# jacobwilliams/splpak

Measured on AMD Instinct MI355X. Metric: fitted points/sec (splcw) + evals/sec (splfe), 3-D 1e7 pts 64^3 nodes, higher is better.
Workload: dtype f64; 1 GPU; C3: 3-D splcw least-squares spline fit, 10000000 weighted scattered points (Park-Miller stream, seed 42), 64x64x64 nodes, xtrap=1, real64; ncol=262144, points_per_gpu=10000000, points_total=10000000, parallelism=single GPU, rccl_ranks=0, refine_steps=2

## Files before the change

### splpak_amd/csrc/ndchol.hip

```cpp
#include "ndstate.hpp"
#include <cstdlib>

namespace splpak {
namespace nd {

hipError_t nd_prefit(splpak_plan *p, hipStream_t st, void *user)
{
    NdState *s = static_cast<NdState *>(user);
    s->tail_pending = false;
    if (s->sch.staged_init && !s->dist) return hipSuccess;
    if (!s->str.sU || !s->ev.evPre || splpak::opt_get("SPLPAK_ND_NO_EARLY_CLEAR")) return hipSuccess;
    long long head = 0;
    if (p->gscratch == s->factor) head = p->gscratch_doubles < s->factor_doubles ? p->gscratch_doubles : s->factor_doubles;
    else if (p->gscratch >= s->factor && p->gscratch < s->factor + s->factor_doubles) return hipSuccess;
    if (head >= s->factor_doubles) return hipSuccess;
    hipError_t e = hipEventRecord(s->ev.evPre, st);
    if (e == hipSuccess) e = hipStreamWaitEvent(s->str.sU, s->ev.evPre, 0);
    const int clear_wgs = splpak::opt_get("SPLPAK_ND_CLEAR_WGS") ? atoi(splpak::opt_get("SPLPAK_ND_CLEAR_WGS")) : 128;
    if (e == hipSuccess) {
        if (clear_wgs > 0) {
            launch_clear(clear_wgs, s->factor + head, s->factor_doubles - head, s->str.sU);
            e = hipGetLastError();
        } else
            e = hipMemsetAsync(s->factor + head, 0, sizeof(double) * (size_t)(s->factor_doubles - head), s->str.sU);
// ... 8 lines not shown
hipError_t nd_assemble(splpak_plan *p, hipStream_t st, void *user)
{
    NdState *s = static_cast<NdState *>(user);
    hipError_t e = hipSuccess;
    if (s->sch.staged_init && !s->dist) {
        if (!s->sch.istarts.empty())
            for (int x : s->sch.istarts[0]) launch_init(s, p->g, p->nst, s->fac.init.l[(size_t)x][0], st);
        return hipGetLastError();
    }
    if (s->tail_pending) {
        if (s->head_doubles > 0) e = hipMemsetAsync(s->factor, 0, sizeof(double) * (size_t)s->head_doubles, st);
        if (e == hipSuccess) e = hipStreamWaitEvent(st, s->ev.evTail, 0);
        s->tail_pending = false;
    } else
        e = hipMemsetAsync(s->factor, 0, sizeof(double) * (size_t)s->factor_doubles, st);
    if (e != hipSuccess) return e;
    launch_assemble(s, p->g, p->nst, st);
    return hipGetLastError();
}

namespace {

struct FactorRun {
    splpak_plan *p;
    NdState *s;
    hipStream_t st, sP, sU, sR;
    int *info_dev;
    double *minpiv_dev;
    CholStats *stats;
    bool timing;
    int pin_rounds;
    int qnext = 0;
    int la_evt = -1;
    bool joined = false, comm_failed = false;
    void syrk(const JobTable<SyrkJob> &tab, const Launch &l, hipStream_t q, bool schur, bool pinned) { launch_syrk(s, tab, l, q, stats, timing, schur, pinned, qnext); }
    void begin();
    void dist_join();
    void potrf_step(const Launch &lp, int k, hipStream_t sC, bool reserved, hipEvent_t after);
    void stage_prep(int i);
    void chain_step(int stg, int k, bool pinned, bool pin_potrf, int prep);
    void root_stage(int stg);
    void run_stage(int i);
    hipError_t end();
};

void hop(hipEvent_t e, hipStream_t from, hipStream_t to) { (void)hipEventRecord(e, from); (void)hipStreamWaitEvent(to, e, 0); }

void zero_block(NdState *s, int x, hipStream_t q) { launch_zero(s->fac.zero, s->fac.zero.l[(size_t)x][0], q); }

void ensure_events(NdState *s, int steps)
{
    for (auto *v : {&s->ev.evT, &s->ev.evI, &s->ev.evW})
        while ((int)v->size() < steps) v->push_back(nd_event(s));
}

void FactorRun::begin()
{
    NdTree &t = s->t;
    if (timing) {
        if (!s->ev.f0) { s->ev.f0 = nd_event(s, true); s->ev.f1 = nd_event(s, true); }
        (void)hipEventRecord(s->ev.f0, st);
    }
    if (s->used && s->ev.evDone) (void)hipStreamWaitEvent(st, s->ev.evDone, 0);
    if (s->zlast_valid) (void)hipStreamWaitEvent(st, s->ev.evZlast, 0);
    if (!s->s_clean && !s->sch.sc.st.empty())
        for (int x : s->sch.starts[0]) zero_block(s, x, st);
    s->s_clean = false;
    if (s->queues) (void)hipMemsetAsync(s->queues, 0, sizeof(int) * ND_QSTRIDE * (size_t)s->nqueues, st);
// ... 46 lines not shown
void FactorRun::potrf_step(const Launch &lp, int k, hipStream_t sC, bool reserved, hipEvent_t after)
{
    if (!reserved) { launch_potrf(s, s->fac.potrf, lp, sC, info_dev, minpiv_dev); return; }
    if (after) (void)hipStreamWaitEvent(sR, after, 0);
    else hop(s->ev.evR0, sC, sR);
    launch_potrf(s, s->fac.potrf, lp, sR, info_dev, minpiv_dev);
    hop(s->ev.evI[(size_t)k], sR, sC);
}

void FactorRun::stage_prep(int i)
{
    for (int x : s->sch.starts[(size_t)i]) zero_block(s, x, sU);
    if (s->sch.staged_init && !s->dist)
        for (int x : s->sch.istarts[(size_t)i]) {
            launch_init(s, p->g, p->nst, s->fac.init.l[(size_t)x][0], sU);
            if (s->sch.sc.st[(size_t)x].dep < 0 && sU != sP) (void)hipEventRecord(s->ev.evP[(size_t)x], sU);
        }
}

void FactorRun::chain_step(int stg, int k, bool pinned, bool pin_potrf, int prep)
{
    FactorTables &F = s->fac;
    const size_t S = (size_t)stg, K = (size_t)k;
    hipStream_t sC = sP;
    const Launch &ls = F.schur.l[S][K], &lf0 = F.fin[0].l[S][K], &lf1 = F.fin[1].l[S][K];
    const bool ahead = pinned && k > 0 && la_evt == k - 1;
    potrf_step(F.potrf.l[S][K], k, sC, pinned && (pin_potrf || ahead), ahead ? s->ev.evW[(size_t)(k - 1)] : nullptr);
    launch_trsm(F.trsm, F.trsm.l[S][K], sC);
    if (prep >= 0) {
        hop(s->ev.evU, sC, sU);
        stage_prep(prep);
    }
    if ((ls.count || lf0.count || lf1.count) && sU != sC) hop(s->ev.evT[K], sC, sU);
    syrk(F.upd, F.upd.l[S][K], sC, false, pinned);
    if (s->sch.chain_la[S] && F.updr.l[S][K].count) {
        if (pinned) {
            (void)hipEventRecord(s->ev.evW[K], sC);
            la_evt = k;
        }
        syrk(F.updr, F.updr.l[S][K], sC, false, pinned);
    }
    syrk(F.updo, F.updo.l[S][K], sC, false, pinned);
    syrk(F.schur, ls, sU, true, pinned);
    syrk(F.fin[0], lf0, sU, true, pinned);
    syrk(F.fin[1], lf1, sU, true, pinned);
}

void FactorRun::root_stage(int stg)
{
    FactorTables &F = s->fac;
    const size_t S = (size_t)stg;
    const int steps = (int)F.potrf.l[S].size();
    ensure_events(s, steps);
    const bool pinned = sR != nullptr && s->nres > 0 && steps > 0 && (int)F.potrf.l[S][0].grid <= pin_rounds * s->nres;
    const bool la = s->sch.lookahead[S] != 0, la2 = s->sch.lookahead[S] == 2;
    for (int k = 0; k < steps; ++k) {
        if (!la) { chain_step(stg, k, pinned, true, -1); continue; }
        const size_t K = (size_t)k;
        const Launch &ltb = F.trsmb.l[S][K], &lur = F.updr.l[S][K];
        potrf_step(F.potrf.l[S][K], k, sP, pinned, nullptr);
        if (ltb.count) {
            if (sU != sP) {
                if (!pinned) (void)hipEventRecord(s->ev.evI[K], sP);
                (void)hipStreamWaitEvent(sU, s->ev.evI[K], 0);
            }
            launch_trsm(F.trsmb, ltb, sU);
        }
        if (!la2 && k > 0 && sU != sP) (void)hipStreamWaitEvent(sP, s->ev.evW[K - 1], 0);
        launch_trsm(F.trsm, F.trsm.l[S][K], sP);
        if (lur.count && sU != sP) hop(s->ev.evT[K], sP, sU);
        if (la2 && k > 0 && sU != sP) (void)hipStreamWaitEvent(sP, s->ev.evW[K - 1], 0);
        syrk(F.upd, F.upd.l[S][K], sP, false, pinned);
        syrk(F.updr, lur, sU, false, pinned);
        if (sU != sP) (void)hipEventRecord(s->ev.evW[K], sU);
    }
    if (sU != sP) hop(s->ev.evU, sU, sP);
}

void FactorRun::run_stage(int i)
{
    FactorTables &F = s->fac;
    const NdStage &S = s->sch.sc.st[(size_t)i];
    if (s->dist && !joined && S.depth <= s->sh.dcut - 1) dist_join();
    auto passes = [&](int k) { return F.schur.l[(size_t)i][(size_t)k].count || F.fin[0].l[(size_t)i][(size_t)k].count || F.fin[1].l[(size_t)i][(size_t)k].count; };
    const int steps = (int)F.potrf.l[(size_t)i].size();
    const bool prep_late = splpak::opt_get("SPLPAK_ND_PREP_EARLY") == nullptr;
    const bool defer = prep_late && i > 0 && i != s->sch.root_stage && sU != sP && steps >= 2 && !passes(0);
    if (i > 0) {
        if (!defer) stage_prep(i);
        if (s->sch.staged_init && !s->dist && S.dep < 0 && sU != sP) (void)hipStreamWaitEvent(sP, s->ev.evP[(size_t)i], 0);
    }
    if (s->sch.fused && S.dep >= 0 && sU != sP) (void)hipStreamWaitEvent(sP, s->ev.evF[(size_t)S.dep], 0);
    la_evt = -1;
    if (i == s->sch.root_stage) { root_stage(i); return; }
    ensure_events(s, steps);
    const bool pinned = sR != nullptr && s->nres > 0 && steps > 0 && ((int)F.potrf.l[(size_t)i][0].grid <= pin_rounds * s->nres || s->sch.chain_la[(size_t)i]);
    const bool unpin_first = splpak::opt_get("SPLPAK_ND_PIN_FIRST") == nullptr;
    bool pass_running = !unpin_first;
    for (int k = 0; k < steps; ++k) {
        chain_step(i, k, pinned, pass_running, k == 0 && defer ? i : -1);
        if (passes(k)) pass_running = true;
    }
    if (s->sch.fused) (void)hipEventRecord(s->ev.evF[(size_t)i], sU);
    else {
        if (sU != sP) hop(s->ev.evU, sU, sP);
// ... 29 lines not shown
    s->s_clean = true;
    (void)hipEventRecord(s->ev.evDone, st);
    s->used = true;
    hipError_t err = hipGetLastError();
    if (timing) {
        (void)hipEventRecord(s->ev.f1, st);
        (void)hipEventSynchronize(s->ev.f1);
        float ms = 0;
        (void)hipEventElapsedTime(&ms, s->ev.f0, s->ev.f1);
        stats->factor_ms = ms;
        for (size_t i = 0; i < (size_t)stats->syrk_launches; ++i) {
            if (hipEventElapsedTime(&ms, s->ev.evA[i], s->ev.evB[i]) == hipSuccess) stats->syrk_ms += ms;
            else (void)hipGetLastError();
        }
    }
    if (err != hipSuccess || top_err != hipSuccess) s->s_clean = false;
    if (comm_failed) return hipErrorUnknown;
    return top_err != hipSuccess ? top_err : err;
}

}

hipError_t nd_factor(splpak_plan *p, int *info_dev, double *minpiv_dev, hipStream_t st, void *user)
{
    NdState *s = static_cast<NdState *>(user);
    const bool timing = p->stats.enabled;
    p->stats = CholStats{};
    p->stats.enabled = timing;
    const bool serial = splpak::opt_get("SPLPAK_NO_LOOKAHEAD") != nullptr;
    FactorRun r{p, s, st, s->str.sP, s->str.sU, s->str.sR, info_dev, minpiv_dev, &p->stats, timing};
    if (serial) r.sP = r.sU = st;
    if (serial || splpak::opt_get("SPLPAK_NO_PANEL_CU")) r.sR = nullptr;
    r.pin_rounds = splpak::opt_get("SPLPAK_ND_PIN_ROUNDS") ? atoi(splpak::opt_get("SPLPAK_ND_PIN_ROUNDS")) : 1;
    r.begin();
    for (int i = 0; i < (int)s->sch.sc.st.size(); ++i) r.run_stage(i);
    return r.end();
}

hipError_t nd_solve(splpak_plan *p, double *x, double *tmp, hipStream_t st, void *user)
{
    (void)tmp;
    NdState *s = static_cast<NdState *>(user);
    NdTree &t = s->t;
    SolveTables &T = s->sol;
    const long long n = t.vec_doubles;
    launch_gather(n, s->rowsrc, x, s->V, st);
    bool comm_failed = false;
    if (s->dist && s->sh.rank != 0)
        for (int id : t.by_depth[(size_t)(s->sh.dcut - 1)]) {
            const NdFront &f = t.fr[(size_t)id];
            (void)hipMemsetAsync(s->V + f.vofs, 0, sizeof(double) * (size_t)f.fp, st);
        }
    const int dlow = s->mdist ? s->top.pt.dcut : 0;
    if (s->mdist) ++s->top.sgen;
    for (int d = t.maxdepth; d >= dlow; --d) {
        if (d < t.maxdepth)
            for (int sl = 0; sl < 2; ++sl) launch_map(T.map, T.map.l[(size_t)(d + 1)][(size_t)sl], false, st);
        if (s->dist && d == s->sh.dcut - 1)
            for (int id : t.by_depth[(size_t)d]) {
                const NdFront &f = t.fr[(size_t)id];
                if (plan_allreduce(p, s->V + f.vofs, f.fp, st) != 0) comm_failed = true;
            }
        const int steps = (int)T.mv.l[(size_t)d].size();
        for (int k = 0; k < steps; ++k) {
            launch_mv(T.mv, T.mv.l[(size_t)d][(size_t)k], st);
            launch_fwd(T.fwd, T.fwd.l[(size_t)d][(size_t)k], st);
// ... 78 lines not shown
```

### splpak_amd/csrc/ndjobs.hip

```cpp
#include "ndstate.hpp"
#include <algorithm>

namespace splpak {
namespace nd {

namespace {

void front_step_jobs(NdState *s, int stg, int id, int k, bool two_level)
{
    NdTree &t = s->t;
    FactorTables &F = s->fac;
    const NdFront &f = t.fr[(size_t)id];
    const bool la = s->sch.lookahead[(size_t)stg] != 0, la2 = s->sch.lookahead[(size_t)stg] == 2, cla = s->sch.chain_la[(size_t)stg] != 0;
    const int schur_kb = s->sch.schur_kb;
    const int g0 = (k / schur_kb) * schur_kb, gend = std::min(g0 + schur_kb, f.nsteps) - 1;
    double *panel = s->factor + s->poff[(size_t)id];
    double *diag = panel + (long long)k * 256 + (long long)k * 256 * f.ld;
    double *below = diag + 256;
    const int nrows = f.fp - (k + 1) * 256;
    double *i16 = s->inv16 + (long long)(s->lblk[(size_t)id] + k) * 4096;
    const int ncols = std::max(1, std::min(256, f.w - k * 256));
    F.potrf.push(PotrfJob{diag, i16, f.ld, f.own0 + k * 256, ncols});
    const int nc = (f.wp - (k + 1) * 256) / 64, nr = nrows / 64;
    if (nrows > 0) {
// ... 9 lines not shown
            tab.push(a, trapezoid_items(c, r));
        };
        auto split = [&](JobTable<SyrkJob> &rect_tab, int nin) {
            const int n4 = std::min(nin, 4);
            trapezoid(F.upd, n4, std::min(nr, 4));
            if (nr > 4) {
                SyrkJob r = proto;
                r.nc = n4; r.nr = nr; r.zinit = -4;
                rect_tab.push(r, (long long)n4 * (nr - 4));
            }
            if (nin > 4) {
                SyrkJob t2 = proto;
                t2.P = below + 256;
                t2.C = below + (long long)256 * f.ld + 256 + (long long)256 * f.ld;
                t2.nc = nin - 4; t2.nr = nr - 4;
                F.updr.push(t2, trapezoid_items(nin - 4, nr - 4));
            }
        };
        if (!la && two_level) {
            const int nc_in = std::min(nc, (gend - k) * 4);
            if (nc_in > 0 && cla) split(F.updr, nc_in);
            else if (nc_in > 0) trapezoid(F.upd, nc_in, nr);
            if (k == gend) {
                SyrkJob o = proto;
                o.P = panel + (long long)(k + 1) * 256 + (long long)g0 * 256 * f.ld;
                o.kb = k - g0 + 1;
                o.nc = nc; o.nr = nr;
                F.updo.push(o, trapezoid_items(nc, nr));
                F.updo.cur.flop += 2.0 * 64 * 64 * 256.0 * o.kb * (double)trapezoid_items(nc, nr);
            }
        } else if (!la)
            trapezoid(F.upd, nc, nr);
        else
            split(la2 ? F.upd : F.updr, nc);
    }
    const int ns = f.hp / 64;
    if (ns > 0 && k == gend) {
        const int kb = k - g0 + 1;
        const int ksl = (k == f.nsteps - 1) ? 4 * ((ncols + 15) / 16) : 64;
        const double jitems = (double)trapezoid_items(ns, ns) - (s->full_diag ? 0.0 : 0.375 * ns);
        const double jflop = 2.0 * 64 * 64 * (256.0 * (kb - 1) + 4.0 * ksl) * jitems;
        const bool boundary = s->mdist && f.depth == s->top.pt.dcut;
        if (s->sch.fused && k == f.nsteps - 1 && f.parent >= 0 && !boundary) {
            const NdFront &pf = t.fr[(size_t)f.parent];
            const int leaf = s->sch.needs[(size_t)id] ? 0 : 1;
            F.fin[f.slot].push(SyrkJob{panel + f.wp + (long long)g0 * 256 * f.ld, s_ptr(s, id), f.ld, s_ld(s, id), ns, ns, 0, kb, ksl, leaf, s->pmap + f.bofs,
                                       s->factor + s->poff[(size_t)f.parent], s_ptr(s, f.parent), pf.ld, s_ld(s, f.parent), pf.wp, f.h},
                               trapezoid_items(ns, ns));
            F.fin[f.slot].cur.flop += jflop;
        } else {
            F.schur.push(SyrkJob{panel + f.wp + (long long)g0 * 256 * f.ld, s_ptr(s, id), f.ld, s_ld(s, id), ns, ns, 0, kb, ksl, 0, nullptr, nullptr, nullptr, 0, 0, 0, 0},
                         trapezoid_items(ns, ns));
            F.schur.cur.flop += jflop;
        }
    }
}

bool stage_jobs(NdState *s, int stg)
{
    NdTree &t = s->t;
    FactorTables &F = s->fac;
    const std::vector<int> &ids = s->sch.sc.st[(size_t)stg].ids;
    F.zero.open();
    for (int id : ids) {
        const NdFront &f = t.fr[(size_t)id];
        if (f.hp == 0 || !s->sch.needs[(size_t)id]) continue;
        const int nt = f.hp / 64;
        F.zero.push(ZeroJob{s_ptr(s, id), s_ld(s, id), nt, 0}, trapezoid_items(nt, nt));
    }
    if (!F.zero.close((size_t)stg, 0)) return false;
    F.init.open();
    for (int id : ids)
        if (s->poff[(size_t)id] >= 0) F.init.push(InitJob{id, 0}, t.fr[(size_t)id].wp);
    if (!F.init.close((size_t)stg, 0)) return false;
    if (s->sch.sc.st[(size_t)stg].depth >= 1 && !s->sch.fused)
        for (int sl = 0; sl < 2; ++sl) {
            F.add.open();
            for (int id : ids) {
                const NdFront &f = t.fr[(size_t)id];
                if (f.slot != sl || f.h == 0) continue;
                const NdFront &p = t.fr[(size_t)f.parent];
                const int nt = f.hp / 64;
                F.add.push(AddJob{s_ptr(s, id), s->pmap + f.bofs, s->factor + s->poff[(size_t)f.parent], s_ptr(s, f.parent), s_ld(s, id), p.ld,
                                  s_ld(s, f.parent), f.h, nt, p.wp, 0},
                           trapezoid_items(nt, nt));
            }
            if (!F.add.close((size_t)stg, (size_t)sl)) return false;
        }
    return true;
}

bool nd_build_factor_jobs(NdState *s)
{
    NdTree &t = s->t;
    FactorTables &F = s->fac;
    const int nstage = (int)s->sch.sc.st.size();
    JobTable<SyrkJob> *const syrk[] = {&F.upd, &F.updr, &F.updo, &F.schur, &F.fin[0], &F.fin[1]};
    s->sch.lookahead.assign((size_t)nstage, 0);
    s->sch.chain_la.assign((size_t)nstage, 0);
    for_each_table(F, [&](auto &tab) { tab.l.assign((size_t)nstage, {}); });
    const bool two_level = splpak::opt_get("SPLPAK_ND_NO_OUTER") == nullptr;
    for (int stg = 0; stg < nstage; ++stg) {
        const std::vector<int> &ids = s->sch.sc.st[(size_t)stg].ids;
        int steps = 0;
        for (int id : ids) steps = std::max(steps, t.fr[(size_t)id].nsteps);
        bool any_schur = false;
        for (int id : ids) any_schur = any_schur || t.fr[(size_t)id].hp > 0;
        const bool la = !any_schur && steps >= 4 && !splpak::opt_get("SPLPAK_ND_NO_ROOT_LOOKAHEAD");
        const bool la2 = la && !(splpak::opt_get("SPLPAK_ND_ROOT_LA") && atoi(splpak::opt_get("SPLPAK_ND_ROOT_LA")) == 1);
        const int cla_blocks = splpak::opt_get("SPLPAK_ND_CHAIN_LA") ? atoi(splpak::opt_get("SPLPAK_ND_CHAIN_LA")) : 8;
        const bool cla = !la && two_level && steps >= 2 && (int)ids.size() <= cla_blocks && !s->mdist;
        s->sch.chain_la[(size_t)stg] = cla ? 1 : 0;
        s->sch.lookahead[(size_t)stg] = la ? (la2 ? 2 : 1) : 0;
        for (int k = 0; k < steps; ++k) {
            F.potrf.open(); F.trsm.open(); F.trsmb.open();
            for (auto *tab : syrk) tab->open();
            for (int id : ids)
                if (k < t.fr[(size_t)id].nsteps) front_step_jobs(s, stg, id, k, two_level);
            const size_t S = (size_t)stg, K = (size_t)k;
            if (!F.potrf.close(S, K) || !F.trsm.close(S, K) || !F.trsmb.close(S, K)) return false;
            for (auto *tab : syrk)
                if (!tab->close(S, K)) return false;
            F.upd.l[S][K].flop = 2.0 * 64 * 64 * 256 * (double)F.upd.l[S][K].grid;
            F.updr.l[S][K].flop = 2.0 * 64 * 64 * 256 * (double)F.updr.l[S][K].grid;
        }
        if (!stage_jobs(s, stg)) return false;
    }
    for (size_t id = 0; id < t.fr.size(); ++id) {
        const NdFront &f = t.fr[id];
        if (!s->mine.empty() && !s->mine[id]) continue;
        for (int k = 0; k < f.nsteps; ++k) {
            const double *diag = s->factor + s->poff[id] + (long long)k * 256 + (long long)k * 256 * f.ld;
            const long long lb = s->lblk[id] + k;
            F.trinv.host.push_back(TrinvJob{diag, s->inv16 + lb * 4096, s->dinv + lb * 65536, s->dinvt + lb * 65536, f.ld});
        }
    }
    F.ntrinv = (int)F.trinv.host.size();
    return true;
}

bool nd_build_solve_jobs(NdState *s)
{
    NdTree &t = s->t;
    SolveTables &T = s->sol;
    const int nd = t.maxdepth + 1;
    for_each_table(T, [&](auto &tab) { tab.l.assign((size_t)nd, {}); });
    long long part_max = 0;
    for (int d = 0; d < nd; ++d) {
        std::vector<int> ids;
        for (int id : t.by_depth[(size_t)d])
            if (s->mine.empty() || s->mine[(size_t)id]) ids.push_back(id);
        int steps = 0;
        for (int id : ids) steps = std::max(steps, t.fr[(size_t)id].nsteps);
        for (int k = 0; k < steps; ++k) {
            T.mv.open(); T.fwd.open(); T.dot.open(); T.bwd.open();
            long long partofs = 0;
// ... 187 lines not shown
```

### splpak_amd/csrc/ndkernels.hip

```cpp
#include "ndstate.hpp"
#include "chol_device.hpp"
#include <hip/hip_ext.h>
#include <cmath>
#include <type_traits>

namespace splpak {
namespace nd {

template <typename J, typename F>
__device__ __forceinline__ int find_job(const J *__restrict__ jobs, int njobs, int b, F &&first)
{
    int lo = 0, hi = njobs - 1;
    while (lo < hi) {
        const int mid = (lo + hi + 1) >> 1;
        if (first(jobs[mid]) <= b) lo = mid;
        else hi = mid - 1;
    }
    return lo;
}

__device__ __forceinline__ double *schur_tile(double *S, long long lds, int ti, int tj, long long &ld)
{
    if (lds >= 0) {
        ld = lds;
// ... 144 lines not shown
                const unsigned ci = nd_cu_index();
                if (resmap[ci >> 5] & (1u << (ci & 31))) skip = atomicAdd(&queue[1], 1) < margin ? 1 : 0;
                s_b[1] = skip;
                s_b[0] = skip ? 0 : atomicAdd(&queue[0], 1);
            }
            __syncthreads();
            if (s_b[1]) {
                __builtin_amdgcn_s_sleep(127);
                __builtin_amdgcn_s_sleep(127);
                return;
            }
            b = s_b[0];
        }
    }
    if constexpr (WGW > 1) b = b * WGW + (int)(threadIdx.x >> 6);
    if (b >= nitems) return;
    const int sub = SPLIT == 1 ? 0 : b % SPLIT;
    if (SPLIT > 1) b /= SPLIT;
    const int m0 = SPLIT == 1 ? 0 : (SPLIT == 4 ? sub : sub >> 2), n0 = SPLIT == 16 ? (sub & 3) : 0;
    const int ji = find_job(jobs, njobs, b, [](const SyrkJob &t) { return t.item0; });
    const SyrkJob j = jobs[ji];
    int tj, ti;
    if (!SCHUR && j.zinit < 0) {
        const int rb = -j.zinit, per = j.nr - rb, it = b - j.item0;
        tj = it / per;
        ti = rb + it - tj * per;
    } else if (xm && j.nc == j.nr)
        panel_decode(b - j.item0, j.nr, tj, ti);
    else
        trapezoid_decode(b - j.item0, j.nr, tj, ti);
    if (tj >= j.nc || ti >= j.nr) return;
    const bool diag = ti == tj;
    if (SPLIT == 16 && diag && n0 < m0) return;
    const int lane = threadIdx.x & 63, l15 = lane & 15, q = lane >> 4;
    constexpr bool COUNTED = !(SCHUR && SPLIT == 4);
    typedef __attribute__((address_space(1))) double gdouble;
    typedef __attribute__((address_space(1))) const int gint;
    typedef typename std::conditional<COUNTED, __attribute__((address_space(1))) const double, const double>::type opnd_t;
    typedef typename std::conditional<COUNTED, gdouble, double>::type ctile_t;
    opnd_t *__restrict__ pJ = (opnd_t *)(j.P + (long long)(tj * 64 + 16 * m0 + l15) + (long long)q * j.ldp);
    opnd_t *__restrict__ pI = (opnd_t *)(j.P + (long long)(ti * 64 + 16 * n0 + l15) + (long long)q * j.ldp);
    long long ldc;
    ctile_t *__restrict__ C = (ctile_t *)schur_tile(j.C, j.ldc, ti, tj, ldc);
    const long long ldp = j.ldp;
    constexpr bool SBASE = COUNTED && SPLIT == 4;
    typedef __attribute__((address_space(1))) const char gcchar;
    auto uniform = [](const double *p) {
        const unsigned long long a = (unsigned long long)p;
        const unsigned lo = __builtin_amdgcn_readfirstlane((unsigned)a), hi = __builtin_amdgcn_readfirstlane((unsigned)(a >> 32));
        return (gcchar *)(((unsigned long long)hi << 32) | lo);
    };
    gcchar *bJ = uniform(j.P + (tj * 64 + 16 * m0)), *bI = uniform(j.P + (ti * 64 + 16 * n0));
    const unsigned lob = ((unsigned)l15 + (unsigned)q * (unsigned)ldp) * 8u;
    d4_t acc[M][N];
#pragma unroll
    for (int m = 0; m < M; ++m)
#pragma unroll
        for (int n = 0; n < N; ++n)
#pragma unroll
            for (int v = 0; v < 4; ++v)
                acc[m][n][v] = (SCHUR && j.zinit) ? 0.0 : __builtin_nontemporal_load(&C[((n0 + n) * 16 + l15) + (long long)((m0 + m) * 16 + q + 4 * v) * ldc]);
    const bool skipu = diag && !full_diag;
    double qa[SD][M], qb[SD][N];
    auto fetch = [&](int slot, int step) {
        const long long off = (long long)(4 * step) * ldp;
        if constexpr (SBASE) {
#pragma unroll
            for (int m = 0; m < M; ++m) qa[slot][m] = *(opnd_t *)(bJ + (off + 16 * m) * 8 + lob);
#pragma unroll
            for (int n = 0; n < N; ++n) qb[slot][n] = *(opnd_t *)(bI + (off + 16 * n) * 8 + lob);
        } else {
#pragma unroll
            for (int m = 0; m < M; ++m) qa[slot][m] = COUNTED ? pJ[off + 16 * m] : -pJ[off + 16 * m];
#pragma unroll
            for (int n = 0; n < N; ++n) qb[slot][n] = pI[off + 16 * n];
        }
    };
#pragma unroll
    for (int d = 0; d < SD; ++d) fetch(d, d);
    if constexpr (COUNTED) __builtin_amdgcn_s_waitcnt(0x0f70);
    constexpr int NSTEP = NBLK / 4;
    static_assert(NSTEP % SD == 0, "queue depth must divide the k-steps");
    const int last = j.kb * NSTEP - 1;
#pragma unroll 1
    for (int h = 0; h < j.kb; ++h) {
        const int base = h * NSTEP;
        const int kend = (h == j.kb - 1) ? j.ksl : NSTEP;
        for (int ks = 0; ks < NSTEP; ks += SD) {
            if (ks >= kend) break;
#pragma unroll
            for (int d = 0; d < SD; ++d) {
#pragma unroll
                for (int m = 0; m < M; ++m)
#pragma unroll
                    for (int n = 0; n < N; ++n) {
                        if (SPLIT == 1 && skipu && m > n) continue;
                        acc[m][n] = __builtin_amdgcn_mfma_f64_16x16x4f64(qa[d][m], qb[d][n], acc[m][n], 0, 0, COUNTED ? 1 : 0);
                    }
                if (ks + d + SD < NSTEP) fetch(d, base + ks + d + SD);
                else {
                    const int nx = base + ks + d + SD;
                    fetch(d, nx < last ? nx : last);
                }
            }
        }
    }
    if (SCHUR && j.pm) {
        constexpr int BM = M < 2 ? M : 2;
        gint *pm = (gint *)j.pm;
        const int hl = j.h - 1;
        int prow[N], pcol[M][4];
#pragma unroll
        for (int n = 0; n < N; ++n) {
            const int r = ti * 64 + (n0 + n) * 16 + l15, t = pm[r < hl ? r : hl];
            prow[n] = r < j.h ? t : -1;
        }
#pragma unroll
        for (int m = 0; m < M; ++m)
#pragma unroll
            for (int v = 0; v < 4; ++v) {
// ... 703 lines not shown
        }
#pragma unroll
        for (int i = 0; i < 4; ++i) s[i] = wave_sum(s[i]);
        if (lane == 0) {
#pragma unroll
            for (int i = 0; i < 4; ++i) x[r0 + i] = s[i];
        }
    }
}

static void potrf_dispatch(int waves, const PotrfJob *jobs, unsigned n, hipStream_t st, int *info_dev, double *minpiv_dev)
{
    if (waves == 4) hipLaunchKernelGGL(nd_potrf_kernel<4>, dim3(n), dim3(256), 0, st, jobs, info_dev, minpiv_dev);
    else if (waves == 8) hipLaunchKernelGGL(nd_potrf_kernel<8>, dim3(n), dim3(512), 0, st, jobs, info_dev, minpiv_dev);
    else hipLaunchKernelGGL(nd_potrf_kernel<16>, dim3(n), dim3(1024), 0, st, jobs, info_dev, minpiv_dev);
}

template <typename J> static void launch_jobs(void (*kernel)(const J *, int), unsigned threads, const JobTable<J> &tab, const Launch &l, hipStream_t st)
{
    if (l.count && l.grid) hipLaunchKernelGGL(kernel, dim3(l.grid), dim3(threads), 0, st, (const J *)(tab.dev + l.first), l.count);
}
template <typename J> static void launch_each(void (*kernel)(const J *), unsigned gx, unsigned threads, const J *jobs, unsigned njobs, hipStream_t st)
{
    if (njobs) hipLaunchKernelGGL(kernel, dim3(gx, njobs), dim3(threads), 0, st, jobs);
}

void launch_potrf(const NdState *s, const JobTable<PotrfJob> &tab, const Launch &l, hipStream_t st, int *info_dev, double *minpiv_dev)
{
    if (l.count) potrf_dispatch(s->potrf_waves, tab.dev + l.first, l.grid, st, info_dev, minpiv_dev);
}
void launch_trsm(const JobTable<TrsmJob> &tab, const Launch &l, hipStream_t st) { launch_jobs(nd_trsm_kernel, 64, tab, l, st); }
void launch_trinv(const TrinvJob *jobs_dev, int n, hipStream_t st) { launch_each(nd_trinv_kernel, NBLK / 16, 64, jobs_dev, (unsigned)n, st); }

void launch_syrk(NdState *s, const JobTable<SyrkJob> &tab, const Launch &l, hipStream_t st, CholStats *stats, bool timing, bool schur,
                 bool pinned, int &qnext)
{
    if (l.count == 0 || l.grid == 0) return;
    hipEvent_t a = nullptr, b = nullptr;
    if (timing && schur) {
        const size_t i = (size_t)stats->syrk_launches;
        while (s->ev.evA.size() <= i) {
            s->ev.evA.push_back(nd_event(s, true));
            s->ev.evB.push_back(nd_event(s, true));
        }
        a = s->ev.evA[i];
        b = s->ev.evB[i];
        stats->syrk_launches += 1;
        stats->syrk_flop += l.flop;
    }
    if (stats) {
        stats->total_flop += l.flop;
        if (schur) {
            stats->bulk_launches += 1;
            stats->bulk_flop += l.flop;
        }
    }
    const bool small_launch = (int)l.grid <= s->small_grid && !s->small_queue;
    int *queue = nullptr;
    int margin = 0;
    if (pinned && s->nres > 0 && qnext < s->nqueues && !small_launch) {
        queue = s->queues + ND_QSTRIDE * (qnext++);
        margin = 256 * s->nres;
    }
    const SyrkJob *jobs = tab.dev + l.first;
    int split = (int)l.grid * 4 <= s->small_grid ? 16 : ((int)l.grid <= s->small_grid ? 4 : 1);
    if (pinned && split > 4) split = 4;
    const int nit = (int)l.grid * split;
    const bool wg4 = split == 1 && (s->wg4 >= 2 || (s->wg4 == 1 && schur));
    unsigned gx = wg4 ? (l.grid + 3) / 4 : l.grid * (unsigned)split;
    if (s->xmode && schur && split == 1 && !wg4 && !queue) gx = (gx + 7u) / 8u * 8u;
    const dim3 grid(gx + (unsigned)margin);
#define ND_SD(SPL) ((SPL) == 16 ? 32 : ((SPL) == 4 ? 16 : 4))
#define ND_SYRK_GO(SCH, SPL, WW)                                                                                               \
    do {                                                                                                                       \
        if (SCH) hipExtLaunchKernelGGL((nd_syrk_kernel<ND_SD(SPL), 2, SCH, SPL, WW>), grid, dim3(64 * WW), 0, st, a, b, 0, jobs, l.count, nit, margin,  \
                                       (const unsigned *)s->resmap, queue, s->full_diag, s->xmode);                            \
        else hipLaunchKernelGGL((nd_syrk_kernel<ND_SD(SPL), 2, SCH, SPL, WW>), grid, dim3(64 * WW), 0, st, jobs, l.count, nit, margin,   \
                                (const unsigned *)s->resmap, queue, s->full_diag, s->xmode);                                  \
    } while (0)
    if (schur) {
        if (split == 16) ND_SYRK_GO(true, 16, 1); else if (split == 4) ND_SYRK_GO(true, 4, 1); else if (wg4) ND_SYRK_GO(true, 1, 4); else ND_SYRK_GO(true, 1, 1);
    } else {
        if (split == 16) ND_SYRK_GO(false, 16, 1); else if (split == 4) ND_SYRK_GO(false, 4, 1); else if (wg4) ND_SYRK_GO(false, 1, 4); else ND_SYRK_GO(false, 1, 1);
    }
#undef ND_SYRK_GO
#undef ND_SD
}

void launch_add(const JobTable<AddJob> &tab, const Launch &l, hipStream_t st) { launch_jobs(nd_extend_add_kernel, 256, tab, l, st); }
void launch_pull(const JobTable<PullJob> &tab, const Launch &l, hipStream_t st) { launch_jobs(nd_pull_add_kernel, 256, tab, l, st); }
void launch_zero(const JobTable<ZeroJob> &tab, const Launch &l, hipStream_t st) { launch_jobs(nd_zero_kernel, 256, tab, l, st); }
void launch_fwd(const JobTable<FwdJob> &tab, const Launch &l, hipStream_t st) { launch_jobs(nd_fwd_kernel, 512, tab, l, st); }
void launch_dot(const JobTable<DotJob> &tab, const Launch &l, hipStream_t st) { launch_jobs(nd_dot_kernel, 256, tab, l, st); }
void launch_mv(const JobTable<MvJob> &tab, const Launch &l, hipStream_t st) { launch_each(nd_mv_kernel, 16, 256, (const MvJob *)(tab.dev + l.first), l.grid, st); }
void launch_bwd(const JobTable<BwdJob> &tab, const Launch &l, hipStream_t st) { launch_each(nd_bwd_kernel, 16, 256, (const BwdJob *)(tab.dev + l.first), l.grid, st); }
void launch_map(const JobTable<MapJob> &tab, const Launch &l, bool take, hipStream_t st)
{
    launch_each(take ? nd_map_kernel<true> : nd_map_kernel<false>, 8, 256, (const MapJob *)(tab.dev + l.first), l.grid, st);
}
// ... 113 lines not shown
```

### splpak_amd/csrc/ndstate.hpp

```cpp
#pragma once
#include "plan.hpp"
#include "ndtree.hpp"
#include <atomic>
#include <memory>
#include <string>
#include <vector>

namespace splpak {

struct NdGroup {
    int R = 1, chunk = 1;
    std::vector<void *> st;
    std::atomic<int> *abort = nullptr;
    std::atomic<int> own_abort{0};
    HostBarrier bar;
    int nseq = 0;
    std::unique_ptr<std::atomic<int>[]> posted, fposted, bposted, subdone;
    std::vector<int> h_info;
    std::vector<double> h_minpiv;
    bool finalized = false;
    int gen = 0;
};

namespace nd {
// ... 43 lines not shown
    J *dev = nullptr;
    std::vector<std::vector<Launch>> l;
    Launch cur;
    long long items = 0;

    void open() { cur = Launch(); cur.first = (int)host.size(); items = 0; }
    void push(J j, long long n = 1)
    {
        if (int *f = first_item(j)) *f = (int)items;
        host.push_back(j);
        items += n;
        ++cur.count;
    }
    bool close(Launch &out, bool sentinel = true)
    {
        if (items > 0x7fffffffLL) { set_error("nested dissection: launch too large"); return false; }
        cur.grid = (unsigned)items;
        J e = end_job((const J *)nullptr);
        if (int *f = first_item(e); f && sentinel && cur.count) { *f = (int)items; host.push_back(e); }
        out = cur;
        return true;
    }
    bool close(size_t r, size_t c, bool sentinel = true)
    {
        if (l[r].size() <= c) l[r].resize(c + 1);
        return close(l[r][c], sentinel);
    }
};

struct FactorTables {
    JobTable<PotrfJob> potrf;
    JobTable<TrsmJob> trsm, trsmb;
    JobTable<SyrkJob> upd;
    JobTable<SyrkJob> updr;
    JobTable<SyrkJob> updo;
    JobTable<SyrkJob> fin[2];
    JobTable<SyrkJob> schur;
    JobTable<TrinvJob> trinv;
    JobTable<AddJob> add;
    JobTable<ZeroJob> zero;
    JobTable<InitJob> init;
    int ntrinv = 0;
};
template <typename F> void for_each_table(FactorTables &T, F &&f)
{
    f(T.potrf); f(T.trsm); f(T.trsmb); f(T.upd); f(T.updr); f(T.updo); f(T.fin[0]); f(T.fin[1]); f(T.schur); f(T.trinv); f(T.add); f(T.zero); f(T.init);
}

struct SolveTables {
    JobTable<MvJob> mv;
    JobTable<FwdJob> fwd;
    JobTable<DotJob> dot;
    JobTable<BwdJob> bwd;
    JobTable<MapJob> map;
};
template <typename F> void for_each_table(SolveTables &T, F &&f) { f(T.mv); f(T.fwd); f(T.dot); f(T.bwd); f(T.map); }

struct Schedule {
    NdSchedule sc;
    std::vector<char> needs;
    std::vector<std::vector<int>> starts;
    std::vector<std::vector<int>> istarts;
    int root_stage = -1;
    int schur_kb = 4;
    std::vector<char> lookahead;
    std::vector<char> chain_la;
    bool fused = true;
    bool staged_init = false;
};

struct Streams {
    hipStream_t sP = nullptr, sU = nullptr, sR = nullptr, sCopy = nullptr;
};

struct Events {
    std::vector<hipEvent_t> all;
    hipEvent_t ev0 = nullptr, evJ = nullptr, evU = nullptr, evZlast = nullptr, evDone = nullptr, evPre = nullptr, evTail = nullptr, evR0 = nullptr;
    hipEvent_t f0 = nullptr, f1 = nullptr;
    std::vector<hipEvent_t> evF;
// ... 110 lines not shown
    return o >= 0 ? s->sarena + o : nullptr;
}
inline long long s_ld(NdState *s, int id) { return nd_schur_ld(s->t.fr[(size_t)id], s->sch.sc.packed); }
inline const TopColDev &top_col(const NdState *q, size_t ti, int J) { return q->top.topcol[(size_t)q->top.tbase[ti] + (size_t)J]; }

bool nd_alloc_bytes(NdState *s, void **ptr, size_t bytes);
void nd_free_bytes(NdState *s, void **ptr);
template <typename T> bool nd_alloc(NdState *s, T **ptr, size_t count) { return nd_alloc_bytes(s, reinterpret_cast<void **>(ptr), (count ? count : 1) * sizeof(T)); }
template <typename T>
bool nd_upload(NdState *s, T **dev, const std::vector<T> &host)
{
    if (!nd_alloc(s, dev, host.size())) return false;
    if (host.empty()) return true;
    return hip_ok(hipMemcpy(*dev, host.data(), sizeof(T) * host.size(), hipMemcpyHostToDevice), "nested dissection: table upload");
}
template <typename T> void nd_free_dev(NdState *s, T **ptr) { nd_free_bytes(s, reinterpret_cast<void **>(ptr)); }

int nd_make_jobs(NdState *s);
bool nd_build_top_jobs(NdState *s);

hipError_t nd_prefit(splpak_plan *p, hipStream_t st, void *user);
hipError_t nd_assemble(splpak_plan *p, hipStream_t st, void *user);
hipError_t nd_factor(splpak_plan *p, int *info_dev, double *minpiv_dev, hipStream_t st, void *user);
hipError_t nd_solve(splpak_plan *p, double *x, double *tmp, hipStream_t st, void *user);
hipError_t nd_top_factor(NdState *s, hipStream_t st, int *info_dev, double *minpiv_dev, CholStats *stats, bool timing);
hipError_t nd_top_pivots(NdState *s, hipStream_t st, int *info_dev, double *minpiv_dev);
hipError_t nd_top_forward(NdState *s, hipStream_t st);
hipError_t nd_top_backward(NdState *s, hipStream_t st);

void launch_potrf(const NdState *s, const JobTable<PotrfJob> &tab, const Launch &l, hipStream_t st, int *info_dev, double *minpiv_dev);
void launch_trsm(const JobTable<TrsmJob> &tab, const Launch &l, hipStream_t st);
void launch_trinv(const TrinvJob *jobs_dev, int n, hipStream_t st);
void launch_syrk(NdState *s, const JobTable<SyrkJob> &tab, const Launch &l, hipStream_t st, CholStats *stats, bool timing, bool schur,
                 bool pinned, int &qnext);
void launch_add(const JobTable<AddJob> &tab, const Launch &l, hipStream_t st);
void launch_pull(const JobTable<PullJob> &tab, const Launch &l, hipStream_t st);
void launch_zero(const JobTable<ZeroJob> &tab, const Launch &l, hipStream_t st);
void launch_init(const NdState *s, const Grid &g, const double *nst, const Launch &l, hipStream_t st);
void launch_assemble(const NdState *s, const Grid &g, const double *nst, hipStream_t st);
void launch_clear(int wgs, double *p, long long n, hipStream_t st);
void launch_tripack(bool pack, double *S, long long lds, int nt, double *img, hipStream_t st);
void launch_flag(const int *info, double *flag, hipStream_t st);
void launch_unflag(int *info, const double *flag, hipStream_t st);
void launch_whoami(unsigned wgs, unsigned *map, hipStream_t st);
void launch_gather(long long n, const int *rowsrc, const double *b, double *V, hipStream_t st);
void launch_scatter(long long n, const int *rowsrc, const double *V, double *x, hipStream_t st);
void launch_map(const JobTable<MapJob> &tab, const Launch &l, bool take, hipStream_t st);
void launch_mv(const JobTable<MvJob> &tab, const Launch &l, hipStream_t st);
void launch_fwd(const JobTable<FwdJob> &tab, const Launch &l, hipStream_t st);
void launch_dot(const JobTable<DotJob> &tab, const Launch &l, hipStream_t st);
void launch_bwd(const JobTable<BwdJob> &tab, const Launch &l, hipStream_t st);
void launch_gather_many(long long n, const int *rowsrc, const BatchPtrs &b, const BatchVec &w, int R, hipStream_t st);
void launch_scatter_many(long long n, const int *rowsrc, const BatchPtrs &x, const BatchVec &w, int R, hipStream_t st);
void launch_map_many(const JobTable<MapJob> &tab, const Launch &l, bool take, const BatchVec &w, int R, hipStream_t st);
void launch_mv_many(const JobTable<MvJob> &tab, const Launch &l, const BatchVec &w, int R, hipStream_t st);
void launch_fwd_many(const JobTable<FwdJob> &tab, const Launch &l, const BatchVec &w, int R, hipStream_t st);
void launch_dot_many(const JobTable<DotJob> &tab, const Launch &l, const BatchVec &w, int R, hipStream_t st);
void launch_bwd_many(const JobTable<BwdJob> &tab, const Launch &l, const BatchVec &w, int R, hipStream_t st);

}
}
```

### splpak_amd/csrc/options.hip

```cpp
#include "options.hpp"

#include <cctype>
#include <cstdlib>
#include <cstring>
#include <mutex>

extern char **environ;

namespace splpak {

namespace {
struct Known { const char *name; int documented; };
const Known KNOWN[] = {
    {"SPLPAK_BIN_ATOMIC", 0},
    {"SPLPAK_DEBUG", 1},
    {"SPLPAK_DEBUG_NO_PEER", 0},
    {"SPLPAK_DEBUG_SUMS", 0},
    {"SPLPAK_DEBUG_TWOEND", 0},
    {"SPLPAK_DIST_CHUNK", 0},
    {"SPLPAK_FIT_GRID_NODE_BLOCK", 0},
    {"SPLPAK_FIT_GRID_REFINE", 1},
    {"SPLPAK_FIT_GRID_SCRATCH_MB", 1},
    {"SPLPAK_FIT_GRID_WEIGHTED_MAXIT", 1},
    {"SPLPAK_GRAM_SCRATCH_MB", 1},
    {"SPLPAK_GRAM_VALU", 0},
    {"SPLPAK_INTEGRATE_SCRATCH_MB", 1},
    {"SPLPAK_MPLAN_BAND", 0},
    {"SPLPAK_MPLAN_RCCL", 1},
    {"SPLPAK_NARROW_BW", 0},
    {"SPLPAK_ND", 1},
    {"SPLPAK_ND_CHAIN_LA", 0},
    {"SPLPAK_ND_CHUNK", 0},
    {"SPLPAK_ND_CLEAR_WGS", 0},
    {"SPLPAK_ND_CUT", 1},
    {"SPLPAK_ND_DIST", 0},
    {"SPLPAK_ND_FULL_DIAG", 0},
    {"SPLPAK_ND_HALVES", 0},
    {"SPLPAK_ND_KB", 1},
    {"SPLPAK_ND_NO_EARLY_CLEAR", 0},
    {"SPLPAK_ND_NO_FUSE", 0},
    {"SPLPAK_ND_NO_OUTER", 0},
    {"SPLPAK_ND_NO_ROOT_LOOKAHEAD", 0},
    {"SPLPAK_ND_PIN_FIRST", 0},
    {"SPLPAK_ND_PIN_ROUNDS", 0},
    {"SPLPAK_ND_POTRF_WAVES", 0},
    {"SPLPAK_ND_PREP_EARLY", 0},
    {"SPLPAK_ND_RES_CUS", 1},
    {"SPLPAK_ND_ROOT_LA", 0},
    {"SPLPAK_ND_SMALL_GRID", 0},
    {"SPLPAK_ND_SMALL_QUEUE", 0},
    {"SPLPAK_ND_SPLIT", 1},
    {"SPLPAK_ND_SQUARE", 0},
    {"SPLPAK_ND_STAGED_INIT", 0},
    {"SPLPAK_ND_WG4", 0},
    {"SPLPAK_ND_XCD", 0},
    {"SPLPAK_NO_LOOKAHEAD", 0},
    {"SPLPAK_NO_PANEL_CU", 0},
    {"SPLPAK_NO_PLAN_CACHE", 1},
    {"SPLPAK_NO_REORDER", 1},
    {"SPLPAK_NO_TWOEND", 0},
    {"SPLPAK_PCG_ALWAYS", 0},
    {"SPLPAK_PCG_ASSEMBLE", 0},
    {"SPLPAK_PCG_EAGER", 0},
    {"SPLPAK_PCG_MAXIT", 1},
// ... 92 lines not shown
```

Measured before the change: 43.62 million points/s.

## Run critical-path panel updates on reserved CUs and split lookahead update table

Moves the root-stage POTRF and the lookahead-critical SYRK update onto the reserved-CU stream when the launch fits the reserved capacity. A new updb table splits the la2 update from the critical upd so the bulk part runs on the main stream. Chain SYRK kernels get raised wave priority and a simplified k-loop. The aim is to shorten the critical dependency chain of the supernodal Cholesky by isolating it from bulk trailing work. The cost is extra event hops and possible contention or starvation on the few reserved CUs.

```diff
diff --git a/splpak_amd/csrc/ndchol.hip b/splpak_amd/csrc/ndchol.hip
--- a/splpak_amd/csrc/ndchol.hip
+++ b/splpak_amd/csrc/ndchol.hip
@@ -64,8 +64,11 @@
     int pin_rounds;
     int qnext = 0;
     int la_evt = -1;
+    bool chain_res = true;
     bool joined = false, comm_failed = false;
     void syrk(const JobTable<SyrkJob> &tab, const Launch &l, hipStream_t q, bool schur, bool pinned) { launch_syrk(s, tab, l, q, stats, timing, schur, pinned, qnext); }
+    bool res_upd(const Launch &l) const { return chain_res && sR && l.count && fits_reserved(s, (long long)l.grid * syrk_split(s, l.grid, true)); }
+    void syrk_res(const JobTable<SyrkJob> &tab, const Launch &l) { launch_syrk(s, tab, l, sR, stats, timing, false, true, qnext, true); }
     void begin();
     void dist_join();
     void potrf_step(const Launch &lp, int k, hipStream_t sC, bool reserved, hipEvent_t after);
@@ -178,10 +181,16 @@
         stage_prep(prep);
     }
     if ((ls.count || lf0.count || lf1.count) && sU != sC) hop(s->ev.evT[K], sC, sU);
-    syrk(F.upd, F.upd.l[S][K], sC, false, pinned);
-    if (s->sch.chain_la[S] && F.updr.l[S][K].count) {
+    const bool la_in = s->sch.chain_la[S] && F.updr.l[S][K].count;
+    const bool upd_res = la_in && pinned && res_upd(F.upd.l[S][K]);
+    if (upd_res) {
+        hop(s->ev.evR0, sC, sR);
+        syrk_res(F.upd, F.upd.l[S][K]);
+    } else
+        syrk(F.upd, F.upd.l[S][K], sC, false, pinned);
+    if (la_in) {
         if (pinned) {
-            (void)hipEventRecord(s->ev.evW[K], sC);
+            (void)hipEventRecord(s->ev.evW[K], upd_res ? sR : sC);
             la_evt = k;
         }
         syrk(F.updr, F.updr.l[S][K], sC, false, pinned);
@@ -200,11 +209,21 @@
     ensure_events(s, steps);
     const bool pinned = sR != nullptr && s->nres > 0 && steps > 0 && (int)F.potrf.l[S][0].grid <= pin_rounds * s->nres;
     const bool la = s->sch.lookahead[S] != 0, la2 = s->sch.lookahead[S] == 2;
+    hipStream_t cur = sP;
+    auto to_res = [&] {
+        if (cur != sR) hop(s->ev.evR0, cur, sR);
+        cur = sR;
+    };
     for (int k = 0; k < steps; ++k) {
         if (!la) { chain_step(stg, k, pinned, true, -1); continue; }
         const size_t K = (size_t)k;
-        const Launch &ltb = F.trsmb.l[S][K], &lur = F.updr.l[S][K];
-        potrf_step(F.potrf.l[S][K], k, sP, pinned, nullptr);
+        const Launch &ltb = F.trsmb.l[S][K], &lu = F.upd.l[S][K], &lub = F.updb.l[S][K], &lur = F.updr.l[S][K];
+        if (pinned) {
+            to_res();
+            launch_potrf(s, F.potrf, F.potrf.l[S][K], sR, info_dev, minpiv_dev);
+            (void)hipEventRecord(s->ev.evI[K], sR);
+        } else
+            launch_potrf(s, F.potrf, F.potrf.l[S][K], sP, info_dev, minpiv_dev);
         if (ltb.count) {
             if (sU != sP) {
                 if (!pinned) (void)hipEventRecord(s->ev.evI[K], sP);
@@ -212,11 +231,20 @@
             }
             launch_trsm(F.trsmb, ltb, sU);
         }
+        if (cur == sR) (void)hipStreamWaitEvent(sP, s->ev.evI[K], 0);
+        cur = sP;
         if (!la2 && k > 0 && sU != sP) (void)hipStreamWaitEvent(sP, s->ev.evW[K - 1], 0);
         launch_trsm(F.trsm, F.trsm.l[S][K], sP);
         if (lur.count && sU != sP) hop(s->ev.evT[K], sP, sU);
-        if (la2 && k > 0 && sU != sP) (void)hipStreamWaitEvent(sP, s->ev.evW[K - 1], 0);
-        syrk(F.upd, F.upd.l[S][K], sP, false, pinned);
+        const bool upd_res = pinned && res_upd(lu);
+        if (upd_res) to_res();
+        if (la2 && k > 0 && sU != sP) (void)hipStreamWaitEvent(cur, s->ev.evW[K - 1], 0);
+        if (upd_res) syrk_res(F.upd, lu);
+        else syrk(F.upd, lu, sP, false, pinned);
+        if (lub.count) {
+            if (upd_res && k > 0 && sU != sP) (void)hipStreamWaitEvent(sP, s->ev.evW[K - 1], 0);
+            syrk(F.updb, lub, sP, false, pinned);
+        }
         syrk(F.updr, lur, sU, false, pinned);
         if (sU != sP) (void)hipEventRecord(s->ev.evW[K], sU);
     }
@@ -312,6 +340,7 @@
     if (serial) r.sP = r.sU = st;
     if (serial || splpak::opt_get("SPLPAK_NO_PANEL_CU")) r.sR = nullptr;
     r.pin_rounds = splpak::opt_get("SPLPAK_ND_PIN_ROUNDS") ? atoi(splpak::opt_get("SPLPAK_ND_PIN_ROUNDS")) : 1;
+    if (const char *e = splpak::opt_get("SPLPAK_ND_CHAIN_ON_RESERVED")) r.chain_res = atoi(e) != 0;
     r.begin();
     for (int i = 0; i < (int)s->sch.sc.st.size(); ++i) r.run_stage(i);
     return r.end();
diff --git a/splpak_amd/csrc/ndjobs.hip b/splpak_amd/csrc/ndjobs.hip
--- a/splpak_amd/csrc/ndjobs.hip
+++ b/splpak_amd/csrc/ndjobs.hip
@@ -65,7 +65,7 @@
         } else if (!la)
             trapezoid(F.upd, nc, nr);
         else
-            split(la2 ? F.upd : F.updr, nc);
+            split(la2 ? F.updb : F.updr, nc);
     }
     const int ns = f.hp / 64;
     if (ns > 0 && k == gend) {
@@ -128,7 +128,7 @@
     NdTree &t = s->t;
     FactorTables &F = s->fac;
     const int nstage = (int)s->sch.sc.st.size();
-    JobTable<SyrkJob> *const syrk[] = {&F.upd, &F.updr, &F.updo, &F.schur, &F.fin[0], &F.fin[1]};
+    JobTable<SyrkJob> *const syrk[] = {&F.upd, &F.updb, &F.updr, &F.updo, &F.schur, &F.fin[0], &F.fin[1]};
     s->sch.lookahead.assign((size_t)nstage, 0);
     s->sch.chain_la.assign((size_t)nstage, 0);
     for_each_table(F, [&](auto &tab) { tab.l.assign((size_t)nstage, {}); });
@@ -155,6 +155,7 @@
             for (auto *tab : syrk)
                 if (!tab->close(S, K)) return false;
             F.upd.l[S][K].flop = 2.0 * 64 * 64 * 256 * (double)F.upd.l[S][K].grid;
+            F.updb.l[S][K].flop = 2.0 * 64 * 64 * 256 * (double)F.updb.l[S][K].grid;
             F.updr.l[S][K].flop = 2.0 * 64 * 64 * 256 * (double)F.updr.l[S][K].grid;
         }
         if (!stage_jobs(s, stg)) return false;
diff --git a/splpak_amd/csrc/ndkernels.hip b/splpak_amd/csrc/ndkernels.hip
--- a/splpak_amd/csrc/ndkernels.hip
+++ b/splpak_amd/csrc/ndkernels.hip
@@ -200,6 +200,8 @@
     if (tj >= j.nc || ti >= j.nr) return;
     const bool diag = ti == tj;
     if (SPLIT == 16 && diag && n0 < m0) return;
+    constexpr bool CHAIN = !SCHUR && SPLIT > 1;
+    if constexpr (CHAIN) __builtin_amdgcn_s_setprio(3);
     const int lane = threadIdx.x & 63, l15 = lane & 15, q = lane >> 4;
     constexpr bool COUNTED = !(SCHUR && SPLIT == 4);
     typedef __attribute__((address_space(1))) double gdouble;
@@ -254,6 +256,21 @@
     for (int h = 0; h < j.kb; ++h) {
         const int base = h * NSTEP;
         const int kend = (h == j.kb - 1) ? j.ksl : NSTEP;
+        if constexpr (CHAIN) {
+#pragma unroll 1
+            for (int ks = 0; ks < kend; ks += SD) {
+#pragma unroll
+                for (int d = 0; d < SD; ++d) {
+#pragma unroll
+                    for (int m = 0; m < M; ++m)
+#pragma unroll
+                        for (int n = 0; n < N; ++n) acc[m][n] = __builtin_amdgcn_mfma_f64_16x16x4f64(qa[d][m], qb[d][n], acc[m][n], 0, 0, 1);
+                    const int nx = base + ks + d + SD;
+                    fetch(d, nx < last ? nx : last);
+                }
+            }
+            continue;
+        }
         for (int ks = 0; ks < NSTEP; ks += SD) {
             if (ks >= kend) break;
 #pragma unroll
@@ -1023,8 +1040,19 @@
 void launch_trsm(const JobTable<TrsmJob> &tab, const Launch &l, hipStream_t st) { launch_jobs(nd_trsm_kernel, 64, tab, l, st); }
 void launch_trinv(const TrinvJob *jobs_dev, int n, hipStream_t st) { launch_each(nd_trinv_kernel, NBLK / 16, 64, jobs_dev, (unsigned)n, st); }
 
+int syrk_split(const NdState *s, unsigned items, bool pinned)
+{
+    const int split = (int)items * 4 <= s->small_grid ? 16 : ((int)items <= s->small_grid ? 4 : 1);
+    return pinned && split > 4 ? 4 : split;
+}
+
+bool fits_reserved(const NdState *s, long long waves)
+{
+    return s->nres > 0 && waves > 0 && waves <= 8LL * s->nres;
+}
+
 void launch_syrk(NdState *s, const JobTable<SyrkJob> &tab, const Launch &l, hipStream_t st, CholStats *stats, bool timing, bool schur,
-                 bool pinned, int &qnext)
+                 bool pinned, int &qnext, bool reserved)
 {
     if (l.count == 0 || l.grid == 0) return;
     hipEvent_t a = nullptr, b = nullptr;
@@ -1046,7 +1074,7 @@
             stats->bulk_flop += l.flop;
         }
     }
-    const bool small_launch = (int)l.grid <= s->small_grid && !s->small_queue;
+    const bool small_launch = reserved || ((int)l.grid <= s->small_grid && !s->small_queue);
     int *queue = nullptr;
     int margin = 0;
     if (pinned && s->nres > 0 && qnext < s->nqueues && !small_launch) {
@@ -1054,8 +1082,7 @@
         margin = 256 * s->nres;
     }
     const SyrkJob *jobs = tab.dev + l.first;
-    int split = (int)l.grid * 4 <= s->small_grid ? 16 : ((int)l.grid <= s->small_grid ? 4 : 1);
-    if (pinned && split > 4) split = 4;
+    const int split = syrk_split(s, l.grid, pinned);
     const int nit = (int)l.grid * split;
     const bool wg4 = split == 1 && (s->wg4 >= 2 || (s->wg4 == 1 && schur));
     unsigned gx = wg4 ? (l.grid + 3) / 4 : l.grid * (unsigned)split;
diff --git a/splpak_amd/csrc/ndstate.hpp b/splpak_amd/csrc/ndstate.hpp
--- a/splpak_amd/csrc/ndstate.hpp
+++ b/splpak_amd/csrc/ndstate.hpp
@@ -99,6 +99,7 @@
     JobTable<PotrfJob> potrf;
     JobTable<TrsmJob> trsm, trsmb;
     JobTable<SyrkJob> upd;
+    JobTable<SyrkJob> updb;
     JobTable<SyrkJob> updr;
     JobTable<SyrkJob> updo;
     JobTable<SyrkJob> fin[2];
@@ -111,7 +112,7 @@
 };
 template <typename F> void for_each_table(FactorTables &T, F &&f)
 {
-    f(T.potrf); f(T.trsm); f(T.trsmb); f(T.upd); f(T.updr); f(T.updo); f(T.fin[0]); f(T.fin[1]); f(T.schur); f(T.trinv); f(T.add); f(T.zero); f(T.init);
+    f(T.potrf); f(T.trsm); f(T.trsmb); f(T.upd); f(T.updb); f(T.updr); f(T.updo); f(T.fin[0]); f(T.fin[1]); f(T.schur); f(T.trinv); f(T.add); f(T.zero); f(T.init);
 }
 
 struct SolveTables {
@@ -288,7 +289,9 @@
 void launch_trsm(const JobTable<TrsmJob> &tab, const Launch &l, hipStream_t st);
 void launch_trinv(const TrinvJob *jobs_dev, int n, hipStream_t st);
 void launch_syrk(NdState *s, const JobTable<SyrkJob> &tab, const Launch &l, hipStream_t st, CholStats *stats, bool timing, bool schur,
-                 bool pinned, int &qnext);
+                 bool pinned, int &qnext, bool reserved = false);
+int syrk_split(const NdState *s, unsigned items, bool pinned);
+bool fits_reserved(const NdState *s, long long waves);
 void launch_add(const JobTable<AddJob> &tab, const Launch &l, hipStream_t st);
 void launch_pull(const JobTable<PullJob> &tab, const Launch &l, hipStream_t st);
 void launch_zero(const JobTable<ZeroJob> &tab, const Launch &l, hipStream_t st);
diff --git a/splpak_amd/csrc/options.hip b/splpak_amd/csrc/options.hip
--- a/splpak_amd/csrc/options.hip
+++ b/splpak_amd/csrc/options.hip
@@ -30,6 +30,7 @@
     {"SPLPAK_NARROW_BW", 0},
     {"SPLPAK_ND", 1},
     {"SPLPAK_ND_CHAIN_LA", 0},
+    {"SPLPAK_ND_CHAIN_ON_RESERVED", 0},
     {"SPLPAK_ND_CHUNK", 0},
     {"SPLPAK_ND_CLEAR_WGS", 0},
     {"SPLPAK_ND_CUT", 1},
```

After: 43.49 million points/s. No clear change (-0.3%).
